# gkaissis/PriMIA

Measured on AMD Instinct MI355X. Metric: images_per_sec, higher is better.
Workload: dtype bf16; 1 GPU; ResNet-18 federated-client training step (fwd+loss+bwd+SGD), batch 256/client, 3x224x224, 1 client per GPU; batch_per_client=256, clients=1, sync_every_n_batch=3, dp_sgd=False

## Files before the change

### primia_amd/csrc/bn.hip

```cpp
#include <stdlib.h>

#include "common.h"

namespace primia {

constexpr int kMaxPartialBlocks = 1024;


template <typename T, typename F, int UNROLL = 0>
__global__ __launch_bounds__(256) void colreduce2_kernel(F f, long M, int C, long rows_per_block,
                                                         float* __restrict__ partials) {
    constexpr int CH = Chunk<T>::N;
    const int tpr = C / CH;
    const int rpp = 256 / tpr;
    const int rg = threadIdx.x / tpr, cc = threadIdx.x % tpr;
    const long r0 = (long)blockIdx.x * rows_per_block;
    long r1 = r0 + rows_per_block;
    if (r1 > M) r1 = M;

    float s1[CH], s2[CH];
#pragma unroll
    for (int i = 0; i < CH; ++i) s1[i] = s2[i] = 0.f;
    if (rg < rpp) {
        F lf = f;
        lf.prepare(cc * CH);
        long r = r0 + rg;
        constexpr int U = UNROLL ? UNROLL : F::kUnroll;
        for (; r + (long)(U - 1) * rpp < r1; r += (long)U * rpp) {
#pragma unroll
            for (int u = 0; u < U; ++u) lf(r + (long)u * rpp, (r + (long)u * rpp) * C + cc * CH, cc * CH, s1, s2);
        }
        for (; r < r1; r += rpp) lf(r, r * C + cc * CH, cc * CH, s1, s2);
    }
    __shared__ float red[2][256 * CH];
    if (rg < rpp) {
#pragma unroll
        for (int i = 0; i < CH; ++i) {
            red[0][rg * C + cc * CH + i] = s1[i];
            red[1][rg * C + cc * CH + i] = s2[i];
        }
    }
    __syncthreads();
    for (int c = threadIdx.x; c < C; c += 256) {
        float a = 0.f, b = 0.f;
        for (int g = 0; g < rpp; ++g) {
            a += red[0][g * C + c];
            b += red[1][g * C + c];
        }
        partials[((long)blockIdx.x * 2 + 0) * C + c] = a;
        partials[((long)blockIdx.x * 2 + 1) * C + c] = b;
    }
}

template <typename T>
struct StatsFn {
    static constexpr int kUnroll = 4;
    const T* y;
    __device__ __forceinline__ void prepare(int) {}
    __device__ __forceinline__ void operator()(long, long off, int c0, float* s1, float* s2) const {
        constexpr int CH = Chunk<T>::N;
        float v[CH];
        Chunk<T>::unpack(*(const u32x4*)(y + off), v);
#pragma unroll
        for (int i = 0; i < CH; ++i) {
            s1[i] += v[i];
            s2[i] += v[i] * v[i];
        }
    }
};

template <typename T>
struct BwdFn {
    static constexpr int kUnroll = 2;
    const T* y;
    const T* z;
    const T* dz;
    const float* mean;
    const float* invstd;
    const float* gamma;
    const float* beta;
    const uint8_t* mask;
    __device__ __forceinline__ void prepare(int) {}
    __device__ __forceinline__ void operator()(long, long off, int c0, float* s1, float* s2) const {
        constexpr int CH = Chunk<T>::N;
        float vy[CH], vg[CH];
        Chunk<T>::unpack(*(const u32x4*)(y + off), vy);
        Chunk<T>::unpack(*(const u32x4*)(dz + off), vg);
        if (z) {
            float vz[CH];
            Chunk<T>::unpack(*(const u32x4*)(z + off), vz);
#pragma unroll
            for (int i = 0; i < CH; ++i) vg[i] = vz[i] > 0.f ? vg[i] : 0.f;
        } else if (mask) {
            const unsigned m = mask[off / CH];
#pragma unroll
            for (int i = 0; i < CH; ++i) vg[i] = (m >> i) & 1u ? vg[i] : 0.f;
        } else if (beta) {
#pragma unroll
            for (int i = 0; i < CH; ++i) {
                const float zz = bn_affine(vy[i], mean[c0 + i], invstd[c0 + i] * gamma[c0 + i], beta[c0 + i]);
                vg[i] = zz > 0.f ? vg[i] : 0.f;
            }
        }
#pragma unroll
        for (int i = 0; i < CH; ++i) {
            const float xh = (vy[i] - mean[c0 + i]) * invstd[c0 + i];
            s1[i] += vg[i];
            s2[i] += vg[i] * xh;
        }
    }
};

constexpr int kFinSlices = 64;
template <int NQ>
__device__ __forceinline__ void fin_gather(const float* __restrict__ partials, int nblk, int C, int c, int ks,
                                           double (&acc)[NQ]) {
    for (int k0 = ks; k0 < nblk; k0 += 8 * kFinSlices) {
        float v[8][NQ];
#pragma unroll
        for (int u = 0; u < 8; ++u) {
            const int k = k0 + u * kFinSlices;
#pragma unroll
            for (int q = 0; q < NQ; ++q) {
                const float t = partials[((long)(k < nblk ? k : nblk - 1) * NQ + q) * C + c];
                v[u][q] = k < nblk ? t : 0.f;
            }
        }
#pragma unroll
        for (int u = 0; u < 8; ++u)
#pragma unroll
            for (int q = 0; q < NQ; ++q) acc[q] += (double)v[u][q];
    }
}

__global__ __launch_bounds__(16 * kFinSlices) void bn_finalize_kernel(const float* __restrict__ partials, int nblk,
                                                          int C, long M, int mode, float eps,
                                                          float momentum, float* out1, float* out2,
                                                          float* running_mean, float* running_var,
                                                          const float* scale2 = nullptr) {
    __shared__ double sa[kFinSlices][17], sb[kFinSlices][17];
    const int cl = threadIdx.x & 15, ks = threadIdx.x >> 4;
    const int c = blockIdx.x * 16 + cl;
    float rm0 = 0.f, rv0 = 0.f, sc2v = 1.f;
    if (ks == 0 && c < C) {
        if (mode == 0 && running_mean) {
            rm0 = running_mean[c];
            rv0 = running_var[c];
        } else if (mode != 0 && scale2) {
            sc2v = scale2[c];
        }
    }
    double acc2[2] = {0.0, 0.0};
    if (c < C) fin_gather<2>(partials, nblk, C, c, ks, acc2);
    double a = acc2[0], b = acc2[1];
    sa[ks][cl] = a;
    sb[ks][cl] = b;
    __syncthreads();
    if (ks >= 4) return;
    for (int k = ks + 4; k < kFinSlices; k += 4) {
        a += sa[k][cl];
        b += sb[k][cl];
    }
    a += __shfl_down(a, 32);
    b += __shfl_down(b, 32);
    a += __shfl_down(a, 16);
    b += __shfl_down(b, 16);
    if (ks != 0 || c >= C) return;
    if (mode == 0) {
        const double mean = a / (double)M;
        double var = b / (double)M - mean * mean;
        if (var < 0.0) var = 0.0;
        out1[c] = (float)mean;
        out2[c] = (float)(1.0 / sqrt(var + (double)eps));
        if (running_mean) {
            const double unb = M > 1 ? var * (double)M / (double)(M - 1) : var;
            running_mean[c] = (float)((1.0 - momentum) * (double)rm0 + (double)momentum * mean);
            running_var[c] = (float)((1.0 - momentum) * (double)rv0 + (double)momentum * unb);
        }
    } else {
        out1[c] = (float)a;
        out2[c] = scale2 ? (float)(b * (double)sc2v) : (float)b;
    }
}

template <typename T>
__global__ __launch_bounds__(16 * kFinSlices) void bn_finalize_pool_kernel(
    const float* __restrict__ partials, int nblk, int C, float* __restrict__ dbeta, float* __restrict__ dgamma,
    const float* __restrict__ gamma, const float* __restrict__ beta, const float* __restrict__ mean,
    const float* __restrict__ invstd, const T* __restrict__ p, const T* __restrict__ dp, const uint8_t* __restrict__ argmax,
    const T* __restrict__ y, int N, int H, int W, int Ho, int Wo) {
    __shared__ double sa[kFinSlices][17], sb[kFinSlices][17];
    __shared__ double sfix[16 * kFinSlices / 64];
    const int cl = threadIdx.x & 15, ks = threadIdx.x >> 4;
    const int c = blockIdx.x * 16 + cl;
    double acc2[2] = {0.0, 0.0};
    if (c < C) fin_gather<2>(partials, nblk, C, c, ks, acc2);
    sa[ks][cl] = acc2[0];
    sb[ks][cl] = acc2[1];
    __syncthreads();
    if (ks == 0 && c < C) {
        double a = 0.0, b = 0.0;
        for (int k = 0; k < kFinSlices; ++k) {
            a += sa[k][cl];
            b += sb[k][cl];
        }
        dbeta[c] = (float)a;
        dgamma[c] = (float)b;
    }
    for (int j = 0; j < 16; ++j) {
        const int cj = blockIdx.x * 16 + j;
        if (cj >= C || pool_xhat_recoverable(gamma[cj], beta[cj])) continue;
        const long Mp = (long)N * Ho * Wo;
        const float mu = mean[cj], is = invstd[cj];
        double t = 0.0;
        for (long r = threadIdx.x; r < Mp; r += blockDim.x) {
            const float pv = Elem<T>::load(p + r * C + cj);
            if (!(pv > 0.f)) continue;
            const int wo = (int)(r % Wo);
            const long q = r / Wo;
            const int ho = (int)(q % Ho), n = (int)(q / Ho);
            const int code = argmax[r * C + cj];
            const int h = 2 * ho - 1 + code / 3, w = 2 * wo - 1 + code % 3;
            const float yv = Elem<T>::load(y + (((long)n * H + h) * W + w) * C + cj);
            t += (double)(Elem<T>::load(dp + r * C + cj) * ((yv - mu) * is));
        }
        for (int o = 32; o > 0; o >>= 1) t += __shfl_down(t, o);
        __syncthreads();
        if ((threadIdx.x & 63) == 0) sfix[threadIdx.x >> 6] = t;
        __syncthreads();
        if (threadIdx.x == 0) {
            double a = 0.0;
            for (int k = 0; k < 16 * kFinSlices / 64; ++k) a += sfix[k];
            dgamma[cj] = (float)a;
        }
    }
}

struct BnInline {
    const float* partials;
    int nblk;
    long M;
    float eps, momentum;
    float* running_mean;
    float* running_var;
    float* save_mean;
    float* save_invstd;
    unsigned* flags;
};

__device__ __forceinline__ void bn_inline_finalize_stats(const BnInline& q, int C, float* lds_mean, float* lds_invstd) {
    const int nfin = (C + 3) >> 2;
    if ((int)blockIdx.x < nfin) {
        __shared__ double sa[kFinSlices][5], sb[kFinSlices][5];
        const int cl = threadIdx.x & 3, ks = threadIdx.x >> 2;
        const int c = blockIdx.x * 4 + cl;
        double acc2[2] = {0.0, 0.0};
        if (c < C) fin_gather<2>(q.partials, q.nblk, C, c, ks, acc2);
        double a = acc2[0], b = acc2[1];
        sa[ks][cl] = a;
        sb[ks][cl] = b;
        __syncthreads();
        if (ks < 4) {
            for (int k = ks + 4; k < kFinSlices; k += 4) {
                a += sa[k][cl];
                b += sb[k][cl];
            }
        }
        __syncthreads();
        if (ks < 4) {
            sa[ks][cl] = a;
            sb[ks][cl] = b;
        }
        __syncthreads();
        if (ks == 0 && c < C) {
            a = (sa[0][cl] + sa[2][cl]) + (sa[1][cl] + sa[3][cl]);
            b = (sb[0][cl] + sb[2][cl]) + (sb[1][cl] + sb[3][cl]);
            const double mean = a / (double)q.M;
            double var = b / (double)q.M - mean * mean;
            if (var < 0.0) var = 0.0;
            __hip_atomic_store(q.save_mean + c, (float)mean, __ATOMIC_RELAXED, __HIP_MEMORY_SCOPE_AGENT);
            __hip_atomic_store(q.save_invstd + c, (float)(1.0 / sqrt(var + (double)q.eps)), __ATOMIC_RELAXED, __HIP_MEMORY_SCOPE_AGENT);
            if (q.running_mean) {
                const double unb = q.M > 1 ? var * (double)q.M / (double)(q.M - 1) : var;
                q.running_mean[c] = (float)((1.0 - q.momentum) * (double)q.running_mean[c] + (double)q.momentum * mean);
                q.running_var[c] = (float)((1.0 - q.momentum) * (double)q.running_var[c] + (double)q.momentum * unb);
            }
        }
        asm volatile("s_waitcnt vmcnt(0)" ::: "memory");
        __syncthreads();
        if (threadIdx.x == 0) __hip_atomic_store(q.flags + blockIdx.x, 1u, __ATOMIC_RELAXED, __HIP_MEMORY_SCOPE_AGENT);
    }
    for (int c = threadIdx.x; c < C; c += blockDim.x) {
        while (__hip_atomic_load(q.flags + (c >> 2), __ATOMIC_RELAXED, __HIP_MEMORY_SCOPE_AGENT) == 0u) __builtin_amdgcn_s_sleep(2);
        asm volatile("" ::: "memory");
        lds_mean[c] = __hip_atomic_load(q.save_mean + c, __ATOMIC_RELAXED, __HIP_MEMORY_SCOPE_AGENT);
        lds_invstd[c] = __hip_atomic_load(q.save_invstd + c, __ATOMIC_RELAXED, __HIP_MEMORY_SCOPE_AGENT);
    }
}

template <typename T>
__global__ __launch_bounds__(256) void bn_apply_kernel(const T* __restrict__ y, const T* __restrict__ res,
                                                       T* __restrict__ z, const float* __restrict__ gamma,
                                                       const float* __restrict__ beta,
                                                       const float* __restrict__ mean,
                                                       const float* __restrict__ invstd_or_var, float eps,
// ... 101 lines not shown
    constexpr int CH = Chunk<T>::N;
    __shared__ float sm[7][512];
    for (int c = threadIdx.x; c < C; c += 256) {
        sm[0][c] = mean[c];
        sm[1][c] = invstd[c];
        sm[2][c] = gamma[c] * invstd[c];
        sm[3][c] = dbeta[c] * inv_m;
        sm[4][c] = dgamma[c] * inv_m;
        sm[5][c] = invstd[c] * gamma[c];
        sm[6][c] = beta ? beta[c] : 0.f;
    }
    __syncthreads();
    const int cpr = C / CH;
    const long stride = (long)gridDim.x * 256;
    for (long q0 = (long)blockIdx.x * 256 + threadIdx.x; q0 < nchunks; q0 += stride * U) {
        u32x4 ry[U], rg[U], rz[U];
        unsigned rm[U];
#pragma unroll
        for (int u = 0; u < U; ++u) {
            const long q = q0 + u * stride;
            const long qc = q < nchunks ? q : q0;
            ry[u] = *(const u32x4*)(y + qc * CH);
            rg[u] = *(const u32x4*)(dz + qc * CH);
            if (z) rz[u] = *(const u32x4*)(z + qc * CH);
            else if (mask) rm[u] = mask[qc];
        }
#pragma unroll
        for (int u = 0; u < U; ++u) {
            const long q = q0 + u * stride;
            if (q >= nchunks) break;
            const int c0 = (int)(q % cpr) * CH;
            float vy[CH], vg[CH];
            Chunk<T>::unpack(ry[u], vy);
            Chunk<T>::unpack(rg[u], vg);
            if (z) {
                float vz[CH];
                Chunk<T>::unpack(rz[u], vz);
#pragma unroll
                for (int i = 0; i < CH; ++i) vg[i] = vz[i] > 0.f ? vg[i] : 0.f;
            } else if (mask) {
                const unsigned m = rm[u];
#pragma unroll
                for (int i = 0; i < CH; ++i) vg[i] = (m >> i) & 1u ? vg[i] : 0.f;
            } else if (beta) {
#pragma unroll
                for (int i = 0; i < CH; ++i) {
                    const float zz = bn_affine(vy[i], sm[0][c0 + i], sm[5][c0 + i], sm[6][c0 + i]);
                    vg[i] = zz > 0.f ? vg[i] : 0.f;
                }
            }
            if (g_out) *(u32x4*)(g_out + q * CH) = Chunk<T>::pack(vg);
#pragma unroll
            for (int i = 0; i < CH; ++i) {
                const float xh = (vy[i] - sm[0][c0 + i]) * sm[1][c0 + i];
                vy[i] = sm[2][c0 + i] * (vg[i] - sm[3][c0 + i] - xh * sm[4][c0 + i]);
            }
            *(u32x4*)(dy + q * CH) = Chunk<T>::pack(vy);
        }
    }
}


template <typename T, int PW, int PH>
__global__ __launch_bounds__(256) void bn_relu_pool_fwd_kernel(const T* __restrict__ y, T* __restrict__ pooled,
                                                               uint8_t* __restrict__ argmax,
                                                               const float* __restrict__ gamma,
                                                               const float* __restrict__ beta,
                                                               const float* __restrict__ mean,
                                                               const float* __restrict__ invstd, int N, int H, int W,
                                                               int C, int Ho, int Wo, int G) {
    constexpr int CH = Chunk<T>::N;
    constexpr int NCOL = 2 * PW + 1, NROW = 2 * PH + 1;
    __shared__ float sm[3][512];
    if (G == 0) {
        for (int c = threadIdx.x; c < C; c += 256) {
            sm[0][c] = mean[c];
            sm[1][c] = invstd[c] * gamma[c];
            sm[2][c] = beta[c];
        }
    }
    __syncthreads();
    const int cpr = C / CH;
    const int Wq = Wo / PW, Hq = Ho / PH;
    const long total = (long)N * Hq * Wq * cpr;
    const long q = (long)blockIdx.x * 256 + threadIdx.x;
    if (q >= total) return;
    const int cc = (int)(q % cpr);
    long t = q / cpr;
    const int wq = (int)(t % Wq);
    t /= Wq;
    const int hq = (int)(t % Hq);
    const int n = (int)(t / Hq);
    const int c0 = cc * CH;
    float best[PH][PW][CH];
    int pos[PH][PW][CH];
#pragma unroll
    for (int kh = 0; kh < PH; ++kh)
#pragma unroll
        for (int k = 0; k < PW; ++k)
#pragma unroll
            for (int i = 0; i < CH; ++i) {
                best[kh][k][i] = 0.f;
                pos[kh][k][i] = -1;
            }
    float mu[CH], sc[CH], be[CH];
#pragma unroll
    for (int i = 0; i < CH; ++i) {
        if (G == 0) {
            mu[i] = sm[0][c0 + i];
            sc[i] = sm[1][c0 + i];
            be[i] = sm[2][c0 + i];
        } else {
            const int ng = n * G + (c0 + i) / (C / G);
            mu[i] = mean[ng];
            sc[i] = invstd[ng] * gamma[c0 + i];
            be[i] = beta[c0 + i];
        }
    }
    const int w0 = wq * PW * 2 - 1;
    const int h0 = hq * PH * 2 - 1;
#pragma unroll
    for (int rr = 0; rr < NROW; ++rr) {
        const int h = h0 + rr;
        if (h < 0 || h >= H) continue;
        const T* row = y + (((long)n * H + h) * W) * C + c0;
        u32x4 raw[NCOL];
#pragma unroll
        for (int col = 0; col < NCOL; ++col) {
            const int w = w0 + col;
            raw[col] = u32x4{0, 0, 0, 0};
            if (w >= 0 && w < W) raw[col] = *(const u32x4*)(row + (long)w * C);
        }
#pragma unroll
        for (int col = 0; col < NCOL; ++col) {
            const int w = w0 + col;
            if (w < 0 || w >= W) continue;
            float v[CH];
            Chunk<T>::unpack(raw[col], v);
#pragma unroll
            for (int i = 0; i < CH; ++i) v[i] = round_to<T>(fmaxf(bn_affine(v[i], mu[i], sc[i], be[i]), 0.f));
#pragma unroll
            for (int kh = 0; kh < PH; ++kh) {
                const int r = rr - 2 * kh;
                if (r < 0 || r > 2) continue;
#pragma unroll
                for (int k = 0; k < PW; ++k) {
                    const int s_ = col - 2 * k;
                    if (s_ < 0 || s_ > 2) continue;
#pragma unroll
                    for (int i = 0; i < CH; ++i) {
                        const float z = v[i];
                        if (pos[kh][k][i] < 0 || z > best[kh][k][i] || z != z) {
                            best[kh][k][i] = z;
                            pos[kh][k][i] = r * 3 + s_;
                        }
                    }
                }
            }
        }
    }
#pragma unroll
    for (int kh = 0; kh < PH; ++kh)
#pragma unroll
        for (int k = 0; k < PW; ++k) {
            const long o = (((long)n * Ho + hq * PH + kh) * Wo + wq * PW + k) * C + c0;
            *(u32x4*)(pooled + o) = Chunk<T>::pack(best[kh][k]);
            uint32_t pk[CH / 4];
#pragma unroll
            for (int j = 0; j < CH / 4; ++j)
                pk[j] = (uint32_t)pos[kh][k][4 * j] | ((uint32_t)pos[kh][k][4 * j + 1] << 8) |
                        ((uint32_t)pos[kh][k][4 * j + 2] << 16) | ((uint32_t)pos[kh][k][4 * j + 3] << 24);
            if constexpr (CH == 8)
                *(u32x2*)(argmax + o) = u32x2{pk[0], pk[1]};
            else
                *(uint32_t*)(argmax + o) = pk[0];
        }
}

template <int PW, int PH>
__global__ __launch_bounds__(1024) void bn_relu_pool_fwd_key_kernel(const bf16* __restrict__ y, bf16* __restrict__ pooled,
                                                                   uint8_t* __restrict__ argmax,
                                                                   const float* __restrict__ gamma,
                                                                   const float* __restrict__ beta,
                                                                   const float* __restrict__ mean,
                                                                   const float* __restrict__ invstd, int N, int H, int W,
                                                                   int C, int Ho, int Wo, int G) {
    constexpr int CH = 8, NCOL = 2 * PW + 1, NROW = 2 * PH + 1;
    __shared__ float sm[3][512];
    const int cpr = C / CH;
    const int Wq = Wo / PW, Hq = Ho / PH;
    const long total = (long)N * Hq * Wq * cpr;
    bool staged = G == 0;
    if (G == 0) {
        for (int c = threadIdx.x; c < C; c += blockDim.x) {
            sm[0][c] = mean[c];
            sm[1][c] = invstd[c] * gamma[c];
            sm[2][c] = beta[c];
        }
    } else {
        const long per_n = (long)Hq * Wq * cpr;
        const long q0 = (long)blockIdx.x * blockDim.x;
        long q1 = q0 + blockDim.x - 1;
        if (q1 >= total) q1 = total - 1;
        const int n0 = (int)(q0 / per_n);
        if (q0 < total && n0 == (int)(q1 / per_n)) {
            staged = true;
            for (int c = threadIdx.x; c < C; c += blockDim.x) {
                const int ng = n0 * G + c / (C / G);
                sm[0][c] = mean[ng];
                sm[1][c] = invstd[ng] * gamma[c];
                sm[2][c] = beta[c];
            }
        }
    }
    __syncthreads();
    const long q = (long)blockIdx.x * blockDim.x + threadIdx.x;
    if (q >= total) return;
    const int cc = (int)(q % cpr);
    long t = q / cpr;
    const int wq = (int)(t % Wq);
    t /= Wq;
    const int hq = (int)(t % Hq);
    const int n = (int)(t / Hq);
    const int c0 = cc * CH;
    unsigned key[PH][PW][CH];
#pragma unroll
    for (int kh = 0; kh < PH; ++kh)
#pragma unroll
        for (int k = 0; k < PW; ++k)
#pragma unroll
            for (int i = 0; i < CH; ++i) key[kh][k][i] = 0u;
    float mu[CH], sc[CH], be[CH];
#pragma unroll
    for (int i = 0; i < CH; ++i) {
        if (staged) {
            mu[i] = sm[0][c0 + i];
            sc[i] = sm[1][c0 + i];
            be[i] = sm[2][c0 + i];
        } else {
            const int ng = n * G + (c0 + i) / (C / G);
            mu[i] = mean[ng];
            sc[i] = invstd[ng] * gamma[c0 + i];
            be[i] = beta[c0 + i];
        }
    }
    const int w0 = wq * PW * 2 - 1;
    const int h0 = hq * PH * 2 - 1;
#pragma unroll
    for (int rr = 0; rr < NROW; ++rr) {
        const int h = h0 + rr;
        if (h < 0 || h >= H) continue;
        const bf16* row = y + (((long)n * H + h) * W) * C + c0;
        u32x4 raw[NCOL];
#pragma unroll
        for (int col = 0; col < NCOL; ++col) {
            const int w = w0 + col;
            raw[col] = u32x4{0, 0, 0, 0};
            if (w >= 0 && w < W) raw[col] = *(const u32x4*)(row + (long)w * C);
        }
#pragma unroll
        for (int col = 0; col < NCOL; ++col) {
            const int w = w0 + col;
            if (w < 0 || w >= W) continue;
            float v[CH];
            Chunk<bf16>::unpack(raw[col], v);
            unsigned zb[CH];
#pragma unroll
            for (int i = 0; i < CH; ++i)
                zb[i] = (unsigned)f32_to_bf16(fmaxf(bn_affine(v[i], mu[i], sc[i], be[i]), 0.f)) & 0x7fffu;
#pragma unroll
            for (int kh = 0; kh < PH; ++kh) {
                const int r = rr - 2 * kh;
                if (r < 0 || r > 2) continue;
#pragma unroll
                for (int k = 0; k < PW; ++k) {
                    const int s_ = col - 2 * k;
                    if (s_ < 0 || s_ > 2) continue;
                    const unsigned tail = 15u - (unsigned)(r * 3 + s_);
#pragma unroll
                    for (int i = 0; i < CH; ++i) {
                        const unsigned cand = (zb[i] << 4) | tail;
                        key[kh][k][i] = cand > key[kh][k][i] ? cand : key[kh][k][i];
                    }
                }
            }
        }
    }
#pragma unroll
    for (int kh = 0; kh < PH; ++kh)
#pragma unroll
        for (int k = 0; k < PW; ++k) {
            const long o = (((long)n * Ho + hq * PH + kh) * Wo + wq * PW + k) * C + c0;
            u32x4 pv;
            uint32_t pk[2];
#pragma unroll
            for (int j = 0; j < 4; ++j) pv[j] = (key[kh][k][2 * j] >> 4) | ((key[kh][k][2 * j + 1] >> 4) << 16);
#pragma unroll
            for (int j = 0; j < 2; ++j)
                pk[j] = (15u - (key[kh][k][4 * j] & 15u)) | ((15u - (key[kh][k][4 * j + 1] & 15u)) << 8) |
                        ((15u - (key[kh][k][4 * j + 2] & 15u)) << 16) | ((15u - (key[kh][k][4 * j + 3] & 15u)) << 24);
            *(u32x4*)(pooled + o) = pv;
            *(u32x2*)(argmax + o) = u32x2{pk[0], pk[1]};
        }
}

template <typename T>
__device__ __forceinline__ void pool_gather(const T* __restrict__ dp, const uint8_t* __restrict__ argmax, int n, int h,
                                            int w, int c0, int C, int Ho, int Wo, float* g) {
    constexpr int CH = Chunk<T>::N;
#pragma unroll
    for (int i = 0; i < CH; ++i) g[i] = 0.f;
    int hoc[2], rc[2], woc[2], sc[2];
    bool hv[2], wv[2];
    hoc[0] = (h + 1) >> 1; rc[0] = h + 1 - 2 * hoc[0]; hv[0] = hoc[0] < Ho;
    hoc[1] = (h - 1) >> 1; rc[1] = 2;                  hv[1] = (h & 1) != 0;
    woc[0] = (w + 1) >> 1; sc[0] = w + 1 - 2 * woc[0]; wv[0] = woc[0] < Wo;
    woc[1] = (w - 1) >> 1; sc[1] = 2;                  wv[1] = (w & 1) != 0;
#pragma unroll
    for (int a = 0; a < 2; ++a)
#pragma unroll
        for (int b = 0; b < 2; ++b) {
            const bool ok = hv[a] && wv[b];
            const int ho = ok ? hoc[a] : 0, wo = ok ? woc[b] : 0;
            const long o = (((long)n * Ho + ho) * Wo + wo) * C + c0;
            float v[CH];
            Chunk<T>::unpack(*(const u32x4*)(dp + o), v);
            const unsigned code = ok ? (unsigned)(rc[a] * 3 + sc[b]) : 0xffu;
            if (CH == 8) {
                const u32x2 m = *(const u32x2*)(argmax + o);
#pragma unroll
                for (int i = 0; i < 4; ++i) {
                    g[i] += ((m[0] >> (8 * i)) & 0xffu) == code ? v[i] : 0.f;
                    g[4 + i] += ((m[1] >> (8 * i)) & 0xffu) == code ? v[4 + i] : 0.f;
                }
            } else {
                const uint32_t m = *(const uint32_t*)(argmax + o);
#pragma unroll
                for (int i = 0; i < CH; ++i) g[i] += ((m >> (8 * i)) & 0xffu) == code ? v[i] : 0.f;
            }
        }
}

template <typename T>
struct PoolScatterFn {
    static constexpr int kUnroll = 4;
    const T* p;
    const T* dp;
    const uint8_t* argmax;
    const T* y;
    const float* mean;
    const float* invstd;
    const float* gamma;
    const float* beta;
    int H, W, C, Ho, Wo;
    float k_beta[Chunk<T>::N], k_rgamma[Chunk<T>::N], k_mean[Chunk<T>::N], k_invstd[Chunk<T>::N];
    bool any_zero_gamma;
    __device__ __forceinline__ void prepare(int c0) {
        any_zero_gamma = false;
#pragma unroll
        for (int i = 0; i < Chunk<T>::N; ++i) {
            const float g = gamma[c0 + i];
            k_beta[i] = beta[c0 + i];
            const bool rec = pool_xhat_recoverable(g, k_beta[i]);
            k_rgamma[i] = rec ? 1.f / g : 0.f;
            k_mean[i] = mean[c0 + i];
            k_invstd[i] = invstd[c0 + i];
            any_zero_gamma |= !rec;
        }
    }
    __device__ __forceinline__ void operator()(long row, long off, int c0, float* s1, float* s2) const {
        constexpr int CH = Chunk<T>::N;
        float vp[CH], vd[CH];
        Chunk<T>::unpack(*(const u32x4*)(p + off), vp);
        Chunk<T>::unpack(*(const u32x4*)(dp + off), vd);
#pragma unroll
        for (int i = 0; i < CH; ++i) {
            const float g = vp[i] > 0.f ? vd[i] : 0.f;
            s1[i] += g;
            s2[i] += g * ((vp[i] - k_beta[i]) * k_rgamma[i]);
        }
        if (any_zero_gamma) {
            const int wo = (int)(row % Wo);
            const long t = row / Wo;
            const int ho = (int)(t % Ho), n = (int)(t / Ho);
#pragma unroll
            for (int i = 0; i < CH; ++i) {
                if (k_rgamma[i] != 0.f || !(vp[i] > 0.f)) continue;
                const int code = argmax[off + i];
                const int h = 2 * ho - 1 + code / 3, w = 2 * wo - 1 + code % 3;
                const float yv = Elem<T>::load(y + (((long)n * H + h) * W + w) * C + c0 + i);
                s2[i] += vd[i] * ((yv - k_mean[i]) * k_invstd[i]);
            }
        }
    }
};

template <typename T>
__global__ __launch_bounds__(256) void bn_relu_pool_bwd_apply_kernel(
    const T* __restrict__ y, const T* __restrict__ dp, const uint8_t* __restrict__ argmax, T* __restrict__ dy,
    const float* __restrict__ gamma, const float* __restrict__ beta, const float* __restrict__ mean,
    const float* __restrict__ invstd, const float* __restrict__ dbeta, const float* __restrict__ dgamma, float inv_m,
    int N, int H, int W, int C, int Ho, int Wo, float rcp_w, float rcp_h) {
    constexpr int CH = Chunk<T>::N;
    __shared__ float sm[7][512];
    for (int c = threadIdx.x; c < C; c += 256) {
        sm[0][c] = mean[c];
        sm[1][c] = invstd[c];
        sm[2][c] = gamma[c] * invstd[c];
        sm[3][c] = dbeta[c] * inv_m;
        sm[4][c] = dgamma[c] * inv_m;
        sm[5][c] = invstd[c] * gamma[c];
        sm[6][c] = beta[c];
    }
    __syncthreads();
    const int cpr = C / CH;
    const long total = (long)N * H * W * cpr;
    const long stride = (long)gridDim.x * 256;
    for (long q = (long)blockIdx.x * 256 + threadIdx.x; q < total; q += stride) {
        const int m = (int)(q / cpr);
        const int c0 = (int)(q - (long)m * cpr) * CH;
        int w = m % W;
        const int t = m / W;
        const int h = t % H, n = t / H;
        float vy[CH], vg[CH];
        Chunk<T>::unpack(*(const u32x4*)(y + q * CH), vy);
        pool_gather<T>(dp, argmax, n, h, w, c0, C, Ho, Wo, vg);
#pragma unroll
        for (int i = 0; i < CH; ++i) {
            const float zz = bn_affine(vy[i], sm[0][c0 + i], sm[5][c0 + i], sm[6][c0 + i]);
            const float gi = zz > 0.f ? vg[i] : 0.f;
            const float xh = (vy[i] - sm[0][c0 + i]) * sm[1][c0 + i];
            vy[i] = sm[2][c0 + i] * (gi - sm[3][c0 + i] - xh * sm[4][c0 + i]);
        }
        *(u32x4*)(dy + q * CH) = Chunk<T>::pack(vy);
    }
}

static inline void reduce_geometry(long M, int C, int& nblk, long& rows_per_block) {
    constexpr long min_rows = 32;
    long nb = (M + min_rows - 1) / min_rows;
    if (nb > kMaxPartialBlocks) nb = kMaxPartialBlocks;
    if (nb < 1) nb = 1;
    rows_per_block = (M + nb - 1) / nb;
    nblk = (int)((M + rows_per_block - 1) / rows_per_block);
}

static inline int stream_blocks(long nchunks) {
    long b = (nchunks + 255) / 256;
    return (int)(b < 2048 ? (b < 1 ? 1 : b) : 2048);
}

template <typename T>
static int bn_fwd_train_impl(const void* y, const void* residual, void* z, const float* gamma,
                             const float* beta, float* running_mean, float* running_var,
                             float* save_mean, float* save_invstd, long M, int C, float eps,
                             float momentum, int relu, float* partials, hipStream_t st) {
    int nblk;
    long rpb;
    reduce_geometry(M, C, nblk, rpb);
    StatsFn<T> f{(const T*)y};
    colreduce2_kernel<T, StatsFn<T>><<<nblk, 256, 0, st>>>(f, M, C, rpb, partials);
    bn_finalize_kernel<<<(C + 15) / 16, 16 * kFinSlices, 0, st>>>(partials, nblk, C, M, 0, eps, momentum, save_mean, save_invstd,
                                           running_mean, running_var);
    const long nchunks = M * C / Chunk<T>::N;
    bn_apply_kernel<T><<<stream_blocks(nchunks), 256, 0, st>>>((const T*)y, (const T*)residual, (T*)z, gamma,
                                                               beta, save_mean, save_invstd, eps, 0, nchunks,
                                                               C, relu);
    return launch_status();
}

template <typename T>
static int bn_bwd_impl(const void* y, const void* z, const void* dz, void* dy, void* g_out,
                       const float* gamma, const float* save_mean, const float* save_invstd,
                       float* dgamma, float* dbeta, long M, int C, int relu, float* partials,
                       hipStream_t st, const float* beta = nullptr, const uint8_t* mask = nullptr) {
    int nblk;
    long rpb;
    reduce_geometry(M, C, nblk, rpb);
    BwdFn<T> f{(const T*)y, relu ? (const T*)z : nullptr, (const T*)dz, save_mean, save_invstd, gamma, beta, mask};
    colreduce2_kernel<T, BwdFn<T>><<<nblk, 256, 0, st>>>(f, M, C, rpb, partials);
    bn_finalize_kernel<<<(C + 15) / 16, 16 * kFinSlices, 0, st>>>(partials, nblk, C, M, 1, 0.f, 0.f, dbeta, dgamma, nullptr, nullptr);
    const long nchunks = M * C / Chunk<T>::N;
    if (nchunks >= 4L * 2048 * 256)
        bn_bwd_apply_kernel<T, 2><<<stream_blocks(nchunks), 256, 0, st>>>(
            (const T*)y, relu ? (const T*)z : nullptr, (const T*)dz, (T*)dy, (T*)g_out, gamma, save_mean,
            save_invstd, dbeta, dgamma, (float)(1.0 / (double)M), nchunks, C, beta, mask);
    else
        bn_bwd_apply_kernel<T><<<stream_blocks(nchunks), 256, 0, st>>>(
            (const T*)y, relu ? (const T*)z : nullptr, (const T*)dz, (T*)dy, (T*)g_out, gamma, save_mean,
            save_invstd, dbeta, dgamma, (float)(1.0 / (double)M), nchunks, C, beta, mask);
    return launch_status();
}

template <typename T>
__global__ __launch_bounds__(256) void bn_bwd_pair_reduce_kernel(const T* __restrict__ y2, const T* __restrict__ yd,
                                                                 const T* __restrict__ dz,
                                                                 const uint8_t* __restrict__ mask,
                                                                 const float* __restrict__ mean2,
                                                                 const float* __restrict__ invstd2,
                                                                 const float* __restrict__ meand,
                                                                 const float* __restrict__ invstdd, long M, int C,
                                                                 long rows_per_block, float* __restrict__ partials) {
    constexpr int CH = Chunk<T>::N;
    const int tpr = C / CH, rpp = 256 / tpr;
    const int rg = threadIdx.x / tpr, cc = threadIdx.x % tpr;
    const long r0 = (long)blockIdx.x * rows_per_block;
    long r1 = r0 + rows_per_block;
    if (r1 > M) r1 = M;
    float s1[CH], s2[CH], s3[CH];
#pragma unroll
    for (int i = 0; i < CH; ++i) s1[i] = s2[i] = s3[i] = 0.f;
    const int c0 = cc * CH;
    if (rg < rpp) {
        for (long r = r0 + rg; r < r1; r += rpp) {
            const long off = r * C + c0;
            float v2[CH], vd[CH], vg[CH];
            Chunk<T>::unpack(*(const u32x4*)(y2 + off), v2);
            Chunk<T>::unpack(*(const u32x4*)(yd + off), vd);
            Chunk<T>::unpack(*(const u32x4*)(dz + off), vg);
            const unsigned m = mask[off / CH];
#pragma unroll
            for (int i = 0; i < CH; ++i) {
                vg[i] = (m >> i) & 1u ? vg[i] : 0.f;
                const float xh2 = (v2[i] - mean2[c0 + i]) * invstd2[c0 + i];
                const float xhd = (vd[i] - meand[c0 + i]) * invstdd[c0 + i];
                s1[i] += vg[i];
                s2[i] += vg[i] * xh2;
                s3[i] += vg[i] * xhd;
            }
        }
    }
    __shared__ float red[3][256 * CH];
    if (rg < rpp) {
#pragma unroll
        for (int i = 0; i < CH; ++i) {
            red[0][rg * C + c0 + i] = s1[i];
            red[1][rg * C + c0 + i] = s2[i];
            red[2][rg * C + c0 + i] = s3[i];
        }
    }
    __syncthreads();
    for (int c = threadIdx.x; c < C; c += 256) {
        float a = 0.f, b = 0.f, d = 0.f;
        for (int g = 0; g < rpp; ++g) {
            a += red[0][g * C + c];
            b += red[1][g * C + c];
            d += red[2][g * C + c];
        }
        partials[((long)blockIdx.x * 3 + 0) * C + c] = a;
        partials[((long)blockIdx.x * 3 + 1) * C + c] = b;
        partials[((long)blockIdx.x * 3 + 2) * C + c] = d;
    }
}

__global__ __launch_bounds__(16 * kFinSlices) void bn_finalize3_kernel(const float* __restrict__ partials, int nblk, int C,
                                                                      float* dbeta2, float* dgamma2, float* dbetad,
                                                                      float* dgammad) {
    __shared__ double sa[kFinSlices][17], sb[kFinSlices][17], sc[kFinSlices][17];
    const int cl = threadIdx.x & 15, ks = threadIdx.x >> 4;
    const int c = blockIdx.x * 16 + cl;
    double acc3[3] = {0.0, 0.0, 0.0};
    if (c < C) fin_gather<3>(partials, nblk, C, c, ks, acc3);
    double a = acc3[0], b = acc3[1], d = acc3[2];
    sa[ks][cl] = a;
    sb[ks][cl] = b;
    sc[ks][cl] = d;
    __syncthreads();
    if (ks >= 4) return;
    for (int k = ks + 4; k < kFinSlices; k += 4) {
        a += sa[k][cl];
        b += sb[k][cl];
        d += sc[k][cl];
    }
    a += __shfl_down(a, 32);
    b += __shfl_down(b, 32);
    d += __shfl_down(d, 32);
    a += __shfl_down(a, 16);
    b += __shfl_down(b, 16);
    d += __shfl_down(d, 16);
    if (ks != 0 || c >= C) return;
    dbeta2[c] = (float)a;
    dgamma2[c] = (float)b;
    dbetad[c] = (float)a;
    dgammad[c] = (float)d;
}

template <typename T>
__global__ __launch_bounds__(256) void bn_bwd_pair_apply_kernel(
    const T* __restrict__ y2, const T* __restrict__ yd, const T* __restrict__ dz, const uint8_t* __restrict__ mask,
    T* __restrict__ dy2, T* __restrict__ dyd, const float* __restrict__ gamma2, const float* __restrict__ mean2,
    const float* __restrict__ invstd2, const float* __restrict__ gammad, const float* __restrict__ meand,
    const float* __restrict__ invstdd, const float* __restrict__ dbeta, const float* __restrict__ dgamma2,
    const float* __restrict__ dgammad, float inv_m, long nchunks, int C) {
    constexpr int CH = Chunk<T>::N;
    __shared__ float sm[9][512];
    for (int c = threadIdx.x; c < C; c += 256) {
        sm[0][c] = mean2[c];
        sm[1][c] = invstd2[c];
        sm[2][c] = gamma2[c] * invstd2[c];
        sm[3][c] = dbeta[c] * inv_m;
        sm[4][c] = dgamma2[c] * inv_m;
        sm[5][c] = meand[c];
        sm[6][c] = invstdd[c];
        sm[7][c] = gammad[c] * invstdd[c];
        sm[8][c] = dgammad[c] * inv_m;
    }
    __syncthreads();
    const int cpr = C / CH;
    const long stride = (long)gridDim.x * 256;
    for (long q = (long)blockIdx.x * 256 + threadIdx.x; q < nchunks; q += stride) {
        const int c0 = (int)(q % cpr) * CH;
        float v2[CH], vd[CH], vg[CH];
        Chunk<T>::unpack(*(const u32x4*)(y2 + q * CH), v2);
        Chunk<T>::unpack(*(const u32x4*)(yd + q * CH), vd);
        Chunk<T>::unpack(*(const u32x4*)(dz + q * CH), vg);
        const unsigned m = mask[q];
#pragma unroll
        for (int i = 0; i < CH; ++i) {
            vg[i] = (m >> i) & 1u ? vg[i] : 0.f;
            const float xh2 = (v2[i] - sm[0][c0 + i]) * sm[1][c0 + i];
            const float xhd = (vd[i] - sm[5][c0 + i]) * sm[6][c0 + i];
            v2[i] = sm[2][c0 + i] * (vg[i] - sm[3][c0 + i] - xh2 * sm[4][c0 + i]);
            vd[i] = sm[7][c0 + i] * (vg[i] - sm[3][c0 + i] - xhd * sm[8][c0 + i]);
        }
        *(u32x4*)(dy2 + q * CH) = Chunk<T>::pack(v2);
        *(u32x4*)(dyd + q * CH) = Chunk<T>::pack(vd);
    }
}

template <typename T>
static int bn_bwd_pair_impl(const void* y2, const void* yd, const void* dz, const uint8_t* mask, void* dy2, void* dyd,
                            const float* gamma2, const float* mean2, const float* invstd2, const float* gammad,
                            const float* meand, const float* invstdd, float* dgamma2, float* dbeta2, float* dgammad,
                            float* dbetad, long M, int C, float* partials, hipStream_t st) {
    int nblk;
    long rpb;
    reduce_geometry(M, C, nblk, rpb);
    bn_bwd_pair_reduce_kernel<T><<<nblk, 256, 0, st>>>((const T*)y2, (const T*)yd, (const T*)dz, mask, mean2, invstd2,
                                                       meand, invstdd, M, C, rpb, partials);
    bn_finalize3_kernel<<<(C + 15) / 16, 16 * kFinSlices, 0, st>>>(partials, nblk, C, dbeta2, dgamma2, dbetad, dgammad);
    const long nchunks = M * C / Chunk<T>::N;
    bn_bwd_pair_apply_kernel<T><<<stream_blocks(nchunks), 256, 0, st>>>(
        (const T*)y2, (const T*)yd, (const T*)dz, mask, (T*)dy2, (T*)dyd, gamma2, mean2, invstd2, gammad, meand,
        invstdd, dbeta2, dgamma2, dgammad, (float)(1.0 / (double)M), nchunks, C);
    return launch_status();
}

template <typename T>
static void launch_bn_relu_pool_fwd(const void* y, void* pooled, uint8_t* argmax, const float* gamma, const float* beta,
                                    const float* mean, const float* invstd, int N, int H, int W, int C, int Ho, int Wo,
                                    hipStream_t st, int G = 0) {
    const int pw = Wo % 2 == 0 ? 2 : 1;
    if constexpr (sizeof(T) == 2) {
        const long ktotal = (long)N * Ho * (Wo / pw) * (C / 8);
        const unsigned kgrid = (unsigned)((ktotal + 255) / 256);
        auto kk = pw == 2 ? bn_relu_pool_fwd_key_kernel<2, 1> : bn_relu_pool_fwd_key_kernel<1, 1>;
        kk<<<kgrid, 256, 0, st>>>((const bf16*)y, (bf16*)pooled, argmax, gamma, beta, mean, invstd, N, H, W, C, Ho, Wo, G);
        return;
    }
    const long total = (long)N * Ho * (Wo / pw) * (C / Chunk<T>::N);
    const unsigned grid = (unsigned)((total + 255) / 256);
    auto kern = pw == 2 ? bn_relu_pool_fwd_kernel<T, 2, 1> : bn_relu_pool_fwd_kernel<T, 1, 1>;
    kern<<<grid, 256, 0, st>>>((const T*)y, (T*)pooled, argmax, gamma, beta, mean, invstd, N, H, W, C, Ho, Wo, G);
}

void launch_gn_relu_pool_fwd(const void* y, void* pooled, uint8_t* argmax, const float* gamma, const float* beta,
                             const float* mean, const float* invstd, int N, int H, int W, int C, int G, int dtype,
                             hipStream_t st) {
    const int Ho = (H + 2 - 3) / 2 + 1, Wo = (W + 2 - 3) / 2 + 1;
    if (dtype == PRIMIA_F32)
        launch_bn_relu_pool_fwd<float>(y, pooled, argmax, gamma, beta, mean, invstd, N, H, W, C, Ho, Wo, st, G);
    else
        launch_bn_relu_pool_fwd<bf16>(y, pooled, argmax, gamma, beta, mean, invstd, N, H, W, C, Ho, Wo, st, G);
}

template <typename T>
static int bn_relu_pool_fwd_impl(const void* y, void* pooled, uint8_t* argmax, const float* gamma, const float* beta,
                                 float* running_mean, float* running_var, float* save_mean, float* save_invstd, int N,
                                 int H, int W, int C, float eps, float momentum, float* partials, hipStream_t st) {
    const long M = (long)N * H * W;
    int nblk;
    long rpb;
    reduce_geometry(M, C, nblk, rpb);
    StatsFn<T> f{(const T*)y};
    colreduce2_kernel<T, StatsFn<T>><<<nblk, 256, 0, st>>>(f, M, C, rpb, partials);
    bn_finalize_kernel<<<(C + 15) / 16, 16 * kFinSlices, 0, st>>>(partials, nblk, C, M, 0, eps, momentum, save_mean, save_invstd,
                                                       running_mean, running_var);
    const int Ho = (H + 2 - 3) / 2 + 1, Wo = (W + 2 - 3) / 2 + 1;
    launch_bn_relu_pool_fwd<T>(y, pooled, argmax, gamma, beta, save_mean, save_invstd, N, H, W, C, Ho, Wo, st);
    return launch_status();
}

template <typename T>
__global__ __launch_bounds__(256) void bn_relu_pool_bwd_apply2x2_kernel(
    const T* __restrict__ y, const T* __restrict__ dp, const uint8_t* __restrict__ argmax, T* __restrict__ dy,
    const float* __restrict__ gamma, const float* __restrict__ beta, const float* __restrict__ mean,
    const float* __restrict__ invstd, const float* __restrict__ dbeta, const float* __restrict__ dgamma, float inv_m,
    int N, int H, int W, int C, int Ho, int Wo) {
    constexpr int CH = Chunk<T>::N;
    __shared__ float sm[7][512];
    for (int c = threadIdx.x; c < C; c += 256) {
        sm[0][c] = mean[c];
        sm[1][c] = invstd[c];
        sm[2][c] = gamma[c] * invstd[c];
        sm[3][c] = dbeta[c] * inv_m;
        sm[4][c] = dgamma[c] * inv_m;
        sm[5][c] = invstd[c] * gamma[c];
        sm[6][c] = beta[c];
    }
    __syncthreads();
    const int cpr = C / CH, H2 = H >> 1, W2 = W >> 1;
    const long total = (long)N * H2 * W2 * cpr;
    const long q = (long)blockIdx.x * 256 + threadIdx.x;
    if (q >= total) return;
    const int c0 = (int)(q % cpr) * CH;
    long t = q / cpr;
    const int b = (int)(t % W2);
    t /= W2;
    const int a = (int)(t % H2), n = (int)(t / H2);
    u32x4 wraw[2][2];
    u32x2 craw[2][2];
#pragma unroll
    for (int di = 0; di < 2; ++di)
#pragma unroll
        for (int dj = 0; dj < 2; ++dj) {
            const bool ok = a + di < Ho && b + dj < Wo;
            const long o = (((long)n * Ho + (ok ? a + di : 0)) * Wo + (ok ? b + dj : 0)) * C + c0;
            wraw[di][dj] = *(const u32x4*)(dp + o);
            if (CH == 8) {
                craw[di][dj] = *(const u32x2*)(argmax + o);
            } else {
                craw[di][dj][0] = *(const uint32_t*)(argmax + o);
                craw[di][dj][1] = 0xffffffffu;
            }
            if (!ok) craw[di][dj] = u32x2{0xffffffffu, 0xffffffffu};
        }
#pragma unroll
    for (int i = 0; i < 2; ++i)
#pragma unroll
        for (int j = 0; j < 2; ++j) {
            const long off = ((((long)n * H + 2 * a + i) * W) + 2 * b + j) * C + c0;
            float vy[CH], g[CH];
            Chunk<T>::unpack(*(const u32x4*)(y + off), vy);
#pragma unroll
            for (int k = 0; k < CH; ++k) g[k] = 0.f;
#pragma unroll
            for (int di = i; di >= 0; --di)
#pragma unroll
                for (int dj = j; dj >= 0; --dj) {
                    const unsigned want = (unsigned)((1 + i - 2 * di) * 3 + (1 + j - 2 * dj));
                    float wv[CH];
                    Chunk<T>::unpack(wraw[di][dj], wv);
#pragma unroll
                    for (int k = 0; k < CH; ++k) {
                        const unsigned code = (craw[di][dj][k >> 2] >> (8 * (k & 3))) & 0xffu;
                        g[k] += code == want ? wv[k] : 0.f;
                    }
                }
#pragma unroll
            for (int k = 0; k < CH; ++k) {
                const float zz = bn_affine(vy[k], sm[0][c0 + k], sm[5][c0 + k], sm[6][c0 + k]);
                const float gi = zz > 0.f ? g[k] : 0.f;
                const float xh = (vy[k] - sm[0][c0 + k]) * sm[1][c0 + k];
                vy[k] = sm[2][c0 + k] * (gi - sm[3][c0 + k] - xh * sm[4][c0 + k]);
            }
            *(u32x4*)(dy + off) = Chunk<T>::pack(vy);
            asm volatile("" ::: "memory");
            __builtin_amdgcn_sched_barrier(0);
        }
}

template <typename T>
static int bn_relu_pool_bwd_impl(const void* y, const void* pooled, const void* dpooled, const uint8_t* argmax,
                                 void* dy, const float* gamma, const float* beta, const float* save_mean,
                                 const float* save_invstd, float* dgamma, float* dbeta, int N, int H, int W, int C,
                                 float* partials, hipStream_t st) {
    const long M = (long)N * H * W;
    const int Ho = (H + 2 - 3) / 2 + 1, Wo = (W + 2 - 3) / 2 + 1;
    const long Mp = (long)N * Ho * Wo;
    int nblk;
    long rpb;
    reduce_geometry(Mp, C, nblk, rpb);
    PoolScatterFn<T> f{(const T*)pooled, (const T*)dpooled, argmax, (const T*)y, save_mean, save_invstd, gamma, beta,
                       H, W, C, Ho, Wo, {}, {}, {}, {}, false};
    colreduce2_kernel<T, PoolScatterFn<T>><<<nblk, 256, 0, st>>>(f, Mp, C, rpb, partials);
    bn_finalize_kernel<<<(C + 15) / 16, 16 * kFinSlices, 0, st>>>(partials, nblk, C, M, 1, 0.f, 0.f, dbeta, dgamma, nullptr, nullptr);
    if (!dy) return launch_status();
    const long nchunks = M * C / Chunk<T>::N;
    if (H % 2 == 0 && W % 2 == 0) {
        const long total = nchunks / 4;
        bn_relu_pool_bwd_apply2x2_kernel<T><<<(unsigned)((total + 255) / 256), 256, 0, st>>>(
            (const T*)y, (const T*)dpooled, argmax, (T*)dy, gamma, beta, save_mean, save_invstd, dbeta, dgamma,
            (float)(1.0 / (double)M), N, H, W, C, Ho, Wo);
    } else {
        bn_relu_pool_bwd_apply_kernel<T><<<stream_blocks(nchunks) * 2, 256, 0, st>>>(
            (const T*)y, (const T*)dpooled, argmax, (T*)dy, gamma, beta, save_mean, save_invstd, dbeta, dgamma,
            (float)(1.0 / (double)M), N, H, W, C, Ho, Wo, 1.0f / (float)W, 1.0f / (float)H);
    }
    return launch_status();
}

}

using namespace primia;

template <typename T>
static int bn_fwd_train_pair_impl(const void* y2, const void* yd, void* z, uint8_t* relu_mask, const float* gamma2,
                                  const float* beta2, float* rm2, float* rv2, float* sm2, float* si2, const float* sums2,
                                  int slots2, const float* gammad, const float* betad, float* rmd, float* rvd, float* smd,
                                  float* sid, const float* sumsd, int slotsd, long M, int C, float eps, float momentum,
                                  float* ws, hipStream_t st) {
    int nblk;
    long rpb;
    reduce_geometry(M, C, nblk, rpb);
    const float* partd = sumsd;
    int nd = slotsd;
    if (!sumsd) {
        StatsFn<T> fd{(const T*)yd};
        colreduce2_kernel<T, StatsFn<T>><<<nblk, 256, 0, st>>>(fd, M, C, rpb, ws);
        partd = ws;
        nd = nblk;
    }
    bn_finalize_kernel<<<(C + 15) / 16, 16 * kFinSlices, 0, st>>>(partd, nd, C, M, 0, eps, momentum, smd, sid, rmd, rvd);
    const float* part = sums2;
    int n2 = slots2;
    if (!sums2) {
        StatsFn<T> f2{(const T*)y2};
        colreduce2_kernel<T, StatsFn<T>><<<nblk, 256, 0, st>>>(f2, M, C, rpb, ws);
        part = ws;
        n2 = nblk;
    }
    bn_finalize_kernel<<<(C + 15) / 16, 16 * kFinSlices, 0, st>>>(part, n2, C, M, 0, eps, momentum, sm2, si2, rm2, rv2);
    const long nchunks = M * C / Chunk<T>::N;
    bn_apply_pair_kernel<T><<<stream_blocks(nchunks), 256, 0, st>>>((const T*)y2, (const T*)yd, (T*)z, gamma2, beta2, sm2,
                                                                    si2, gammad, betad, smd, sid, nchunks, C, relu_mask);
    return launch_status();
}

extern "C" {

int64_t primia_bn_workspace_bytes(int64_t M, int C) {
    (void)M;
    return (int64_t)kMaxPartialBlocks * 2 * C * sizeof(float);
}

int primia_bn_fwd_train(const void* y, const void* residual, void* z, const float* gamma,
                        const float* beta, float* running_mean, float* running_var,
                        float* save_mean, float* save_invstd, int64_t M, int C, float eps,
                        float momentum, int relu, void* workspace, int64_t workspace_bytes,
                        int dtype, primia_stream_t stream) {
    PRIMIA_REQUIRE(y && z && gamma && beta && save_mean && save_invstd && workspace);
    PRIMIA_REQUIRE((running_mean == nullptr) == (running_var == nullptr));
    PRIMIA_REQUIRE(bn_shape_ok(M, C, dtype));
    if (workspace_bytes < primia_bn_workspace_bytes(M, C)) return PRIMIA_ERR_WORKSPACE;
    hipStream_t st = (hipStream_t)stream;
    if (dtype == PRIMIA_F32)
        return bn_fwd_train_impl<float>(y, residual, z, gamma, beta, running_mean, running_var, save_mean,
                                        save_invstd, M, C, eps, momentum, relu, (float*)workspace, st);
    if (dtype == PRIMIA_BF16)
        return bn_fwd_train_impl<bf16>(y, residual, z, gamma, beta, running_mean, running_var, save_mean,
                                       save_invstd, M, C, eps, momentum, relu, (float*)workspace, st);
    return PRIMIA_ERR_ARG;
}

int primia_bn_fwd_train_from_sums(const void* y, const void* residual, void* z, const float* gamma,
                                  const float* beta, float* running_mean, float* running_var, float* save_mean,
                                  float* save_invstd, const float* sums, int slots, int64_t M, int C, float eps,
                                  float momentum, int relu, int dtype, primia_stream_t stream) {
    PRIMIA_REQUIRE(y && z && gamma && beta && save_mean && save_invstd && sums && slots >= 1);
    PRIMIA_REQUIRE((running_mean == nullptr) == (running_var == nullptr));
    PRIMIA_REQUIRE(bn_shape_ok(M, C, dtype));
    hipStream_t st = (hipStream_t)stream;
    bn_finalize_kernel<<<(C + 15) / 16, 16 * kFinSlices, 0, st>>>(sums, slots, C, M, 0, eps, momentum, save_mean, save_invstd,
                                                       running_mean, running_var);
    if (dtype == PRIMIA_F32) {
        const long nchunks = M * C / 4;
        bn_apply_kernel<float><<<stream_blocks(nchunks), 256, 0, st>>>((const float*)y, (const float*)residual,
                                                                       (float*)z, gamma, beta, save_mean, save_invstd,
                                                                       eps, 0, nchunks, C, relu);
    } else if (dtype == PRIMIA_BF16) {
        const long nchunks = M * C / 8;
        bn_apply_kernel<bf16><<<stream_blocks(nchunks), 256, 0, st>>>((const bf16*)y, (const bf16*)residual, (bf16*)z,
                                                                      gamma, beta, save_mean, save_invstd, eps, 0,
                                                                      nchunks, C, relu);
    } else {
        return PRIMIA_ERR_ARG;
    }
    return launch_status();
}

int primia_bn_fwd_train_apply_inline(const void* y, const void* residual, void* z, uint8_t* relu_mask, const float* gamma,
                                     const float* beta, float* running_mean, float* running_var, float* save_mean,
                                     float* save_invstd, const float* sums, int slots, int64_t M, int C, float eps,
                                     float momentum, int relu, uint32_t* flags, int dtype, primia_stream_t stream) {
    PRIMIA_REQUIRE(y && z && gamma && beta && save_mean && save_invstd && sums && slots >= 1 && flags);
    PRIMIA_REQUIRE((running_mean == nullptr) == (running_var == nullptr));
    PRIMIA_REQUIRE(bn_shape_ok(M, C, dtype));
    hipStream_t st = (hipStream_t)stream;
    const long nchunks = M * C / (dtype == PRIMIA_F32 ? 4 : 8);
    const int grid = stream_blocks(nchunks);
    if (relu_mask) relu = 1;
    if (grid < (C + 3) / 4) {
        bn_finalize_kernel<<<(C + 15) / 16, 16 * kFinSlices, 0, st>>>(sums, slots, C, M, 0, eps, momentum, save_mean, save_invstd,
                                                           running_mean, running_var);
        if (dtype == PRIMIA_F32)
            bn_apply_kernel<float><<<grid, 256, 0, st>>>((const float*)y, (const float*)residual, (float*)z, gamma, beta, save_mean,
                                                          save_invstd, eps, 0, nchunks, C, relu, relu_mask);
        else
            bn_apply_kernel<bf16><<<grid, 256, 0, st>>>((const bf16*)y, (const bf16*)residual, (bf16*)z, gamma, beta, save_mean,
                                                         save_invstd, eps, 0, nchunks, C, relu, relu_mask);
        return launch_status();
    }
    BnInline q{sums, slots, (long)M, eps, momentum, running_mean, running_var, save_mean, save_invstd, flags};
    if (dtype == PRIMIA_F32)
        bn_apply_kernel<float><<<grid, 256, 0, st>>>((const float*)y, (const float*)residual, (float*)z, gamma, beta, save_mean,
                                                      save_invstd, eps, 0, nchunks, C, relu, relu_mask, q);
    else if (dtype == PRIMIA_BF16)
        bn_apply_kernel<bf16><<<grid, 256, 0, st>>>((const bf16*)y, (const bf16*)residual, (bf16*)z, gamma, beta, save_mean,
                                                     save_invstd, eps, 0, nchunks, C, relu, relu_mask, q);
    else
        return PRIMIA_ERR_ARG;
    return launch_status();
}

int primia_bn_fwd_eval(const void* y, const void* residual, void* z, const float* gamma,
                       const float* beta, const float* running_mean, const float* running_var,
                       int64_t M, int C, float eps, int relu, int dtype, primia_stream_t stream) {
    PRIMIA_REQUIRE(y && z && gamma && beta && running_mean && running_var);
    PRIMIA_REQUIRE(bn_shape_ok(M, C, dtype));
    hipStream_t st = (hipStream_t)stream;
    if (dtype == PRIMIA_F32) {
        const long nchunks = M * C / 4;
        bn_apply_kernel<float><<<stream_blocks(nchunks), 256, 0, st>>>(
            (const float*)y, (const float*)residual, (float*)z, gamma, beta, running_mean, running_var, eps, 1,
            nchunks, C, relu);
    } else if (dtype == PRIMIA_BF16) {
        const long nchunks = M * C / 8;
        bn_apply_kernel<bf16><<<stream_blocks(nchunks), 256, 0, st>>>(
            (const bf16*)y, (const bf16*)residual, (bf16*)z, gamma, beta, running_mean, running_var, eps, 1,
            nchunks, C, relu);
    } else {
        return PRIMIA_ERR_ARG;
    }
    return launch_status();
}

int primia_bn_fwd_eval_mask(const void* y, const void* residual, void* z, uint8_t* relu_mask, const float* gamma,
                            const float* beta, const float* running_mean, const float* running_var, int64_t M, int C,
                            float eps, int dtype, primia_stream_t stream) {
    PRIMIA_REQUIRE(y && z && relu_mask && gamma && beta && running_mean && running_var);
    PRIMIA_REQUIRE(bn_shape_ok(M, C, dtype));
    hipStream_t st = (hipStream_t)stream;
    if (dtype == PRIMIA_F32) {
        const long nchunks = M * C / 4;
        bn_apply_kernel<float><<<stream_blocks(nchunks), 256, 0, st>>>(
            (const float*)y, (const float*)residual, (float*)z, gamma, beta, running_mean, running_var, eps, 1,
// ... 303 lines not shown
```

### primia_amd/csrc/options.h

```cpp
#pragma once

namespace primia {

#define PRIMIA_OPTIONS(X)                                                                                              \
    X(lh2, 1)                                        \
    X(lh2_bm, 0)                                      \
    X(lh4, 1)                \
    X(c64_blocks, 512)                                         \
    X(c64_dbg, 0)                      \
    X(c64_stages, 4)                                                      \
    X(s2lh, 1)               \
    X(s2lh_dbg, 0)

enum OptId : int {
#define PRIMIA_OPT_ENUM(name, def) kOpt_##name,
    PRIMIA_OPTIONS(PRIMIA_OPT_ENUM)
#undef PRIMIA_OPT_ENUM
        kOptCount
};

extern int g_options[kOptCount];

inline int opt(OptId id) { return __atomic_load_n(&g_options[id], __ATOMIC_RELAXED); }

}

#define PRIMIA_OPT(name) (::primia::opt(::primia::kOpt_##name))
```

Measured before the change: 54510 images/s.

## Add strip-mined BN+ReLU+maxpool forward kernel reusing overlapping input rows

Adds a bf16 kernel for the fused BN-affine, ReLU and 3x3/stride-2 maxpool forward. Each thread walks a vertical strip of output rows and carries the transformed shared boundary input row in registers. Per-channel BN parameters are staged in shared memory per image. This avoids re-reading and re-transforming the overlapping pooling-window row and cuts redundant global loads. In exchange there are fewer threads, so less parallelism, more registers and serial row iteration. The kernel is chosen by a thread-count heuristic and can be overridden by a new option.

```diff
diff --git a/primia_amd/csrc/bn.hip b/primia_amd/csrc/bn.hip
--- a/primia_amd/csrc/bn.hip
+++ b/primia_amd/csrc/bn.hip
@@ -1,6 +1,7 @@
 #include <stdlib.h>
 
 #include "common.h"
+#include "options.h"
 
 namespace primia {
 
@@ -708,6 +709,144 @@
             *(u32x4*)(pooled + o) = pv;
             *(u32x2*)(argmax + o) = u32x2{pk[0], pk[1]};
         }
+}
+
+template <int PW>
+__global__ __launch_bounds__(256) void bn_relu_pool_fwd_key_strip_kernel(
+    const bf16* __restrict__ y, bf16* __restrict__ pooled, uint8_t* __restrict__ argmax, const float* __restrict__ gamma,
+    const float* __restrict__ beta, const float* __restrict__ mean, const float* __restrict__ invstd, int N, int H, int W,
+    int C, int Ho, int Wo, int G, int seg, int bpi) {
+    constexpr int CH = 8, NCOL = 2 * PW + 1;
+    __shared__ float sm[3][512];
+    const int cpr = C / CH;
+    const int Wq = Wo / PW, nseg = (Ho + seg - 1) / seg;
+    const int n = blockIdx.x / bpi;
+    for (int c = threadIdx.x; c < C; c += blockDim.x) {
+        const int ng = G == 0 ? c : n * G + c / (C / G);
+        sm[0][c] = mean[ng];
+        sm[1][c] = invstd[ng] * gamma[c];
+        sm[2][c] = beta[c];
+    }
+    __syncthreads();
+    const int q = (blockIdx.x % bpi) * blockDim.x + threadIdx.x;
+    if (q >= nseg * Wq * cpr) return;
+    const int cc = q % cpr;
+    int t = q / cpr;
+    const int wq = t % Wq;
+    const int sg = t / Wq;
+    const int c0 = cc * CH;
+    float mu[CH], sc[CH], be[CH];
+#pragma unroll
+    for (int i = 0; i < CH; ++i) {
+        mu[i] = sm[0][c0 + i];
+        sc[i] = sm[1][c0 + i];
+        be[i] = sm[2][c0 + i];
+    }
+    const int w0 = wq * PW * 2 - 1;
+    const int ho0 = sg * seg;
+    const int ho1 = ho0 + seg < Ho ? ho0 + seg : Ho;
+    const bf16* img = y + (long)n * H * W * C + c0;
+    bool cv[NCOL];
+#pragma unroll
+    for (int col = 0; col < NCOL; ++col) cv[col] = w0 + col >= 0 && w0 + col < W;
+
+    auto load_row = [&](int h, u32x4* raw) {
+        const bf16* row = img + (long)h * W * C;
+#pragma unroll
+        for (int col = 0; col < NCOL; ++col) {
+            raw[col] = u32x4{0, 0, 0, 0};
+            if (cv[col]) raw[col] = *(const u32x4*)(row + (long)(w0 + col) * C);
+        }
+    };
+    auto transform = [&](const u32x4& raw, unsigned* zb) {
+        float v[CH];
+        Chunk<bf16>::unpack(raw, v);
+#pragma unroll
+        for (int i = 0; i < CH; ++i)
+            zb[i] = (unsigned)f32_to_bf16(fmaxf(bn_affine(v[i], mu[i], sc[i], be[i]), 0.f)) & 0x7fffu;
+    };
+
+    unsigned carry[NCOL][CH / 2];
+    if (ho0 > 0) {
+        u32x4 raw[NCOL];
+        load_row(2 * ho0 - 1, raw);
+#pragma unroll
+        for (int col = 0; col < NCOL; ++col) {
+            unsigned zb[CH];
+            transform(raw[col], zb);
+#pragma unroll
+            for (int j = 0; j < CH / 2; ++j) carry[col][j] = zb[2 * j] | (zb[2 * j + 1] << 16);
+        }
+    }
+    for (int ho = ho0; ho < ho1; ++ho) {
+        unsigned key[PW][CH];
+#pragma unroll
+        for (int k = 0; k < PW; ++k)
+#pragma unroll
+            for (int i = 0; i < CH; ++i) key[k][i] = 0u;
+        const bool hb = 2 * ho + 1 < H;
+        u32x4 ra[NCOL], rb[NCOL];
+        load_row(2 * ho, ra);
+        load_row(hb ? 2 * ho + 1 : 2 * ho, rb);
+        if (ho > 0) {
+#pragma unroll
+            for (int col = 0; col < NCOL; ++col) {
+                if (!cv[col]) continue;
+#pragma unroll
+                for (int k = 0; k < PW; ++k) {
+                    const int s_ = col - 2 * k;
+                    if (s_ < 0 || s_ > 2) continue;
+                    const unsigned tail = 15u - (unsigned)s_;
+#pragma unroll
+                    for (int j = 0; j < CH / 2; ++j) {
+                        const unsigned lo = ((carry[col][j] & 0xffffu) << 4) | tail;
+                        const unsigned hi = ((carry[col][j] >> 16) << 4) | tail;
+                        key[k][2 * j] = lo > key[k][2 * j] ? lo : key[k][2 * j];
+                        key[k][2 * j + 1] = hi > key[k][2 * j + 1] ? hi : key[k][2 * j + 1];
+                    }
+                }
+            }
+        }
+#pragma unroll
+        for (int r = 1; r <= 2; ++r) {
+            if (r == 2 && !hb) break;
+#pragma unroll
+            for (int col = 0; col < NCOL; ++col) {
+                if (!cv[col]) continue;
+                unsigned zb[CH];
+                transform(r == 1 ? ra[col] : rb[col], zb);
+#pragma unroll
+                for (int k = 0; k < PW; ++k) {
+                    const int s_ = col - 2 * k;
+                    if (s_ < 0 || s_ > 2) continue;
+                    const unsigned tail = 15u - (unsigned)(r * 3 + s_);
+#pragma unroll
+                    for (int i = 0; i < CH; ++i) {
+                        const unsigned cand = (zb[i] << 4) | tail;
+                        key[k][i] = cand > key[k][i] ? cand : key[k][i];
+                    }
+                }
+                if (r == 2) {
+#pragma unroll
+                    for (int j = 0; j < CH / 2; ++j) carry[col][j] = zb[2 * j] | (zb[2 * j + 1] << 16);
+                }
+            }
+        }
+#pragma unroll
+        for (int k = 0; k < PW; ++k) {
+            const long o = (((long)n * Ho + ho) * Wo + wq * PW + k) * C + c0;
+            u32x4 pv;
+            uint32_t pk[2];
+#pragma unroll
+            for (int j = 0; j < 4; ++j) pv[j] = (key[k][2 * j] >> 4) | ((key[k][2 * j + 1] >> 4) << 16);
+#pragma unroll
+            for (int j = 0; j < 2; ++j)
+                pk[j] = (15u - (key[k][4 * j] & 15u)) | ((15u - (key[k][4 * j + 1] & 15u)) << 8) |
+                        ((15u - (key[k][4 * j + 2] & 15u)) << 16) | ((15u - (key[k][4 * j + 3] & 15u)) << 24);
+            *(u32x4*)(pooled + o) = pv;
+            *(u32x2*)(argmax + o) = u32x2{pk[0], pk[1]};
+        }
+    }
 }
 
 template <typename T>
@@ -1052,12 +1191,31 @@
     return launch_status();
 }
 
+static constexpr int kPoolSeg = 7;
+static constexpr long kPoolStripMinThreads = 114688;
+static int pool_strip_seg(int N, int Ho, int Wq, int cpr) {
+    const int o = PRIMIA_OPT(pool_seg);
+    if (o != 0) return o > 0 ? o : 0;
+    if (Ho < 2 * kPoolSeg) return 0;
+    const long threads = (long)N * ((Ho + kPoolSeg - 1) / kPoolSeg) * Wq * cpr;
+    return threads >= kPoolStripMinThreads ? kPoolSeg : 0;
+}
+
 template <typename T>
 static void launch_bn_relu_pool_fwd(const void* y, void* pooled, uint8_t* argmax, const float* gamma, const float* beta,
                                     const float* mean, const float* invstd, int N, int H, int W, int C, int Ho, int Wo,
                                     hipStream_t st, int G = 0) {
     const int pw = Wo % 2 == 0 ? 2 : 1;
     if constexpr (sizeof(T) == 2) {
+        const int seg = pool_strip_seg(N, Ho, Wo / pw, C / 8);
+        if (seg > 0) {
+            const int per_n = ((Ho + seg - 1) / seg) * (Wo / pw) * (C / 8);
+            const int bpi = (per_n + 255) / 256;
+            auto ks = pw == 2 ? bn_relu_pool_fwd_key_strip_kernel<2> : bn_relu_pool_fwd_key_strip_kernel<1>;
+            ks<<<(unsigned)N * bpi, 256, 0, st>>>((const bf16*)y, (bf16*)pooled, argmax, gamma, beta, mean, invstd, N, H, W, C,
+                                                  Ho, Wo, G, seg, bpi);
+            return;
+        }
         const long ktotal = (long)N * Ho * (Wo / pw) * (C / 8);
         const unsigned kgrid = (unsigned)((ktotal + 255) / 256);
         auto kk = pw == 2 ? bn_relu_pool_fwd_key_kernel<2, 1> : bn_relu_pool_fwd_key_kernel<1, 1>;
diff --git a/primia_amd/csrc/options.h b/primia_amd/csrc/options.h
--- a/primia_amd/csrc/options.h
+++ b/primia_amd/csrc/options.h
@@ -10,7 +10,8 @@
     X(c64_dbg, 0)                      \
     X(c64_stages, 4)                                                      \
     X(s2lh, 1)               \
-    X(s2lh_dbg, 0)
+    X(s2lh_dbg, 0)           \
+    X(pool_seg, 0)
 
 enum OptId : int {
 #define PRIMIA_OPT_ENUM(name, def) kOpt_##name,
```

Result: no change. 54880 images/s (median of 6 runs) (+0.7%).
